# aalto-speech/AaltoASR

Hardware: AMD Instinct MI355X
Metric: frames/sec GMM log-lik (39-d, 50k Gauss) + MFCC, 1/2/4/8 MI355X (higher is better)
Workload: dtype f32 (2-term fp16 split on the matrix cores, f32 accumulate); 1 GPU; configs[2]: full MFCC chain (FFT -> mel -> log -> DCT -> delta/delta-delta, CMS, normalisation) + 50000-Gaussian scoring + 2-byte LNA codes on 1 h of synthetic 16 kHz audio as 360 x 10 s utterances (449280 frames), int16 samples resident in HBM; dim=39, gaussians=50000, states=3125, gpus_flag=1

## Files before the change

aaltoasr_amd/capi.py:

```python
from __future__ import annotations

import ctypes as C
import os
import re
from typing import Optional

import numpy as np

HERE = os.path.dirname(os.path.abspath(__file__))
LIB_PATH = os.path.join(os.environ.get("AASR_LIBDIR") or os.path.join(HERE, "lib"), "libaasr.so")
HEADER_PATH = os.path.join(HERE, "..", "include", "aasr.h")

AASR_OK = 0
AASR_ERR_INVALID = -1
AASR_ERR_UNSUPPORTED = -2
AASR_ERR_NO_DEVICE = -3
AASR_ERR_IO = -4
AASR_ERR_SHORT_AUDIO = -5


class AasrError(RuntimeError):
    def __init__(self, code: int, msg: str):
        super().__init__("aasr status %d: %s" % (code, msg))
        self.code = code
# ... 368 lines not shown
    L.aasr_gmm_score_f64.argtypes = [vp, vp, i64, vp]
    L.aasr_gmm_get_precision.argtypes = [vp]
    L.aasr_gmm_effective_precision.argtypes = [vp]
    L.aasr_gmm_precision_states.argtypes = [vp, C.POINTER(i64), C.POINTER(i64)]
    L.aasr_free.argtypes = [vp]
    L.aasr_free.restype = None
    L.aasr_feat_get_parameters.argtypes = [vp, cp, C.POINTER(C.c_void_p), C.POINTER(i64)]
    L.aasr_feat_num_modules.argtypes = [vp]
    L.aasr_feat_module_name.argtypes = [vp, C.c_int]
    L.aasr_feat_module_name.restype = cp
    L.aasr_feat_module_type.argtypes = [vp, C.c_int]
    L.aasr_feat_module_type.restype = cp
    L.aasr_gmm_score_pitch_ok.argtypes = [vp]
    L.aasr_gmm_score_dev_pitched.argtypes = [vp, vp, i64, vp, i64, vp]
    L.aasr_lna_encode_dev_pitched.argtypes = [vp, i64, i64, i32, C.c_int, C.c_int, vp, vp, vp]
    L.aasr_feat_write_config.argtypes = [vp, C.POINTER(C.c_void_p), C.POINTER(i64)]
    L.aasr_recipe_read.argtypes = [cp, i32, i32, C.POINTER(C.c_void_p), C.POINTER(i64)]
    L.aasr_recipe_read_all.argtypes = [cp, i32, i32, i32, C.POINTER(C.c_void_p), C.POINTER(i64)]
    L.aasr_audio_read.argtypes = [vp, cp, C.POINTER(C.POINTER(C.c_int16)), C.POINTER(i64),
                                  C.POINTER(i32)]


def check(status: int) -> None:
    if status != AASR_OK:
        raise AasrError(status, lib().aasr_last_error().decode("utf-8", "replace"))


def _ptr(a) -> int:
    if a is None:
        return None
# ... 245 lines not shown
                                       _stream_handle(stream)))

    def score_scratch_floats(self, F: int) -> int:
        return lib().aasr_gmm_score_scratch_floats(self._h, F)

    def score_lna_dev(self, d_frames, d_scratch, d_bytes, normalize: bool = True, lnabytes: int = 2, stream=None) -> None:
        check(lib().aasr_gmm_score_lna_dev(self._h, d_frames.data_ptr(), d_frames.shape[0], int(normalize), lnabytes,
                                           d_scratch.data_ptr(), d_bytes.data_ptr(), _stream_handle(stream)))

    def score_pitch_ok(self) -> bool:
        return bool(lib().aasr_gmm_score_pitch_ok(self._h))

    def score_dev_pitched(self, d_frames, d_out, pitch: int, stream=None) -> None:
        check(lib().aasr_gmm_score_dev_pitched(self._h, _ptr(d_frames), d_frames.shape[0], _ptr(d_out),
                                               pitch, _stream_handle(stream)))

    def gauss_loglik(self, frames: np.ndarray) -> np.ndarray:
        frames = np.ascontiguousarray(frames, np.float32)
        self._check_frames(frames)
        out = np.empty((frames.shape[0], self.num_gaussians), np.float32)
        check(lib().aasr_gmm_gauss_loglik(self._h, _ptr(frames), frames.shape[0], _ptr(out)))
        return out


def lna_encode(state_loglik: np.ndarray, normalize: bool = True, lnabytes: int = 2):
    x = np.ascontiguousarray(state_loglik, np.float32)
    F, S = x.shape
    lp = np.empty((F, S), np.float32)
    by = np.empty((F, S * lnabytes), np.uint8)
    check(lib().aasr_lna_encode(_ptr(x), F, S, int(normalize), lnabytes, _ptr(lp), _ptr(by)))
# ... 1707 lines not shown
```

aaltoasr_amd/csrc/capi.cc:

```cpp
#include <cstdarg>
#include <cstdlib>
#include <cstring>
#include <vector>

#include "common.h"
#include "feat.h"
#include "gmm.h"
#include "pipeline.h"

namespace aasr {

std::string &last_error() {
  static thread_local std::string msg;
  return msg;
}

aasr_status fail(aasr_status code, const char *fmt, ...) {
  char buf[1024];
  va_list ap;
  va_start(ap, fmt);
  vsnprintf(buf, sizeof buf, fmt, ap);
  va_end(ap);
  last_error() = buf;
  return code;
// ... 440 lines not shown
  });
}

int aasr_gmm_score_pitch_ok(const aasr_gmm *h) { return h && gmm_score_pitch_ok(h) ? 1 : 0; }

aasr_status aasr_gmm_score_dev_pitched(aasr_gmm *h, const float *d_frames, int64_t F,
                                       float *d_state_loglik, int64_t pitch, void *stream) {
  return guarded([&] {
    if (!h || (F > 0 && (!d_frames || !d_state_loglik)))
      raise(AASR_ERR_INVALID, "aasr_gmm_score_dev_pitched: null argument");
    if (pitch < h->S) raise(AASR_ERR_INVALID, "aasr_gmm_score_dev_pitched: pitch %ld < %ld states", (long)pitch, (long)h->S);
    gmm_score_launch_pitched(h, d_frames, F, d_state_loglik, pitch, (hipStream_t)stream);
  });
}

aasr_status aasr_lna_encode(const float *state_loglik, int64_t F, int32_t S, int normalize,
                            int lnabytes, float *lp_out, uint8_t *bytes_out) {
  return guarded([&] {
    if (lnabytes != 2 && lnabytes != 4)
      raise(AASR_ERR_INVALID, "lnabytes must be 2 or 4, got %d", lnabytes);
    if (S <= 0) raise(AASR_ERR_INVALID, "aasr_lna_encode: S must be positive");
    if (F <= 0) return;
    if (!state_loglik) raise(AASR_ERR_INVALID, "aasr_lna_encode: null input");
    require_device();
    size_t n = (size_t)F * S;
    DevBuf<float> d_in, d_lp;
    DevBuf<uint8_t> d_by;
    d_in.upload(state_loglik, n);
    if (lp_out) d_lp.alloc(n);
    if (bytes_out) d_by.alloc(n * lnabytes);
// ... 68 lines not shown
```

aaltoasr_amd/csrc/gmm.h:

```cpp
#pragma once
#include <cmath>
#include <cstdint>
#include <string>
#include <functional>
#include <memory>
#include <vector>

#include "common.h"

namespace aasr {

struct HostModel {
  int dim = 0;
  int64_t G = 0;
  std::vector<double> mean, var;
  std::vector<double> cov;
  std::vector<uint8_t> is_full;
  bool any_full() const { return !is_full.empty(); }
  std::vector<double> gauss_bias;
  int n_transforms = 0;
  std::vector<int32_t> g2t;
  std::vector<double> xform;
  double logw_bias = 0;
  double logw(size_t k) const {
// ... 264 lines not shown
  aasr::DevBuf<float> dim_part_x, dim_part_ll;
  aasr::DevBuf<int32_t> dim_mix_off, dim_mix_idx;
  aasr::DevBuf<float> dim_mix_logw;
  std::unique_ptr<aasr_gmm> pool_view;
  std::vector<std::unique_ptr<aasr_gmm>> class_models;
  std::vector<aasr::DevBuf<double>> class_a, class_b;
  std::vector<double> class_logdet;
  aasr::DevBuf<float> class_scratch, class_xframes;
  std::shared_ptr<void> utt_scratch;
  std::shared_ptr<void> recipe_scratch;
  aasr::DevBuf<double> xf_a, xf_b;
  aasr::DevBuf<float> d_xframes;
  aasr::ClusterState cl;
  aasr::DevBuf<float> d_frames, d_out;
  mutable aasr::DevBuf<uint32_t> fop_scratch;
};

namespace aasr {
void gmm_build(aasr_gmm *g, const HostModel &m);
void gmm_set_transforms(aasr_gmm *g, int32_t n_transforms, const int32_t *gauss_to_transform, const double *W);
void gmm_build_pool(aasr_gmm *g);
void gmm_dim_split_score(aasr_gmm *g, const float *d_frames, int64_t F, float *d_out, bool per_gaussian, hipStream_t stream,
                         const unsigned long long *maskw = nullptr, int c1 = 0, const int32_t *gclus = nullptr,
                         bool frames_adapted = false);
void gmm_build_pool_centred(aasr_gmm *g);
void gmm_build_f64(aasr_gmm *g, bool any_dim = false);
void gmm_cluster_score_f64_launch(aasr_gmm *g, const double *d_frames, const double *d_members, int64_t F,
                                  double *d_out, int linear, double det, hipStream_t stream);
void gmm_f64_masked_launch(aasr_gmm *g, const double *d_members, int64_t F, double *d_out, int linear, double det,
                           const int32_t *crow, const unsigned long long *maskw, int c1, const double *ll64,
// ... 6 lines not shown
void gmm_build_tracks(aasr_gmm *g, bool grouped);
void gmm_probe_f16x2(aasr_gmm *g);
void gmm_plan_engine_parts(aasr_gmm *g);
bool gmm_engine_parts_active(const aasr_gmm *g);
bool gmm_engine_parts_clustered(const aasr_gmm *g);
void gmm_scatter_columns(const float *dense, int64_t F, int64_t n, float *out, int64_t pitch, hipStream_t stream);
void gmm_add_bias_nofloor(float *d_out, int64_t n, float bias, hipStream_t stream);
void gmm_gather_engine_columns(const aasr_gmm *g, const float *rows, int64_t F, int64_t in_pitch, float *out, int64_t out_pitch,
                               hipStream_t stream);
int64_t gmm_engine_pitch(const aasr_gmm *g);
int64_t gmm_engine_pitch_max(const aasr_gmm *g);
const int32_t *gmm_engine_colmap(const aasr_gmm *g);
void gmm_score_launch_engine(aasr_gmm *g, const float *d_frames, int64_t F, float *d_out, int64_t pitch, hipStream_t stream);
void lna_encode_launch(const float *d_loglik, int64_t F, int S, int normalize, int lnabytes, float *d_lp,
                       uint8_t *d_bytes, hipStream_t stream, int64_t in_pitch, const int32_t *d_colmap = nullptr);
void gmm_build_centred(aasr_gmm *g);
void gmm_build_fullcov(aasr_gmm *g);
void gmm_full_launch(aasr_gmm *g, const float *d_frames, int64_t F, float *d_out,
                     hipStream_t stream);
bool gmm_score_pitch_ok(const aasr_gmm *g);
void gmm_score_launch_pitched(aasr_gmm *g, const float *d_frames, int64_t F, float *d_out, int64_t pitch,
                              hipStream_t stream);
void gmm_score_launch(aasr_gmm *g, const float *d_frames, int64_t F,
                      float *d_out, hipStream_t stream);
void gmm_gauss_launch(aasr_gmm *g, const float *d_frames, int64_t F,
                      float *d_out, hipStream_t stream);
void gmm_set_clustering(aasr_gmm *g, int32_t n_clusters, int64_t n_pairs,
                        const int32_t *gauss_index, const int32_t *cluster_index);
void gmm_read_clustering(aasr_gmm *g, const char *path);
void gmm_set_clustering_min_evals(aasr_gmm *g, double min_clusters, double min_gaussians);
// ... 18 lines not shown
```

aaltoasr_amd/csrc/gmm_score.hip:

```cpp
#include <hip/hip_runtime.h>
#include <mutex>
#include <unordered_map>

#include <cmath>
#include <cstdlib>

#include "gmm_score_common.h"

namespace aasr {

static bool launch_bf16(const aasr_gmm *g, const TrackLayout &L, const float *d_frames, int64_t F,
                        float *d_out, hipStream_t stream, const ClusterArgs *cl = nullptr, int64_t pitch = 0) {
  if (g->precision == AASR_PREC_F16X2 && L.a16h.p && launch_split<2>(g, L, d_frames, F, d_out, stream, cl, pitch))
    return true;
  return launch_split<3>(g, L, d_frames, F, d_out, stream, cl, pitch);
}

namespace {
struct ProbeCache {
  std::mutex mu;
  std::unordered_map<uint64_t, std::vector<int32_t>> verdicts;
  int64_t runs = 0, hits = 0;
};
ProbeCache &probe_cache() {
// ... 431 lines not shown

static bool engine_parts_public(const aasr_gmm *g);
bool gmm_score_pitch_ok(const aasr_gmm *g) {
  if (!g->dim_parts.empty()) return false;
  if (engine_parts_public(g)) return true;
  if (g->cl.enabled && gmm_engine_parts_clustered(g)) return true;
  if (g->host.factor_path() || g->class_routing || g->precision == AASR_PREC_F64) return false;
  if (g->hyb_enabled && g->cl.enabled) return false;
  if (g->ill_conditioned) return g->centred_ok && !g->cl.enabled && (g->layout_mask & 4);
  if (g->cl.enabled && !gmm_cluster_pitch_ok(g)) return false;
  if ((g->layout_mask & 3) != 3) return false;
  const TrackLayout &L = g->paired.ok ? g->paired : g->tracks;
  return (g->precision == AASR_PREC_F32 || g->precision == AASR_PREC_BF16X3 || g->precision == AASR_PREC_F16X2) && L.ok;
}

bool gmm_engine_parts_active(const aasr_gmm *g) {
  return !g->engine_parts.empty() && g->precision == AASR_PREC_F16X2 && g->use_bf16x3 && !g->cl.enabled &&
         !g->class_routing && g->dim_parts.empty() && (g->layout_mask & 3) == 3;
}

bool gmm_engine_parts_clustered(const aasr_gmm *g) {
  return !g->engine_parts.empty() && g->cl.enabled && g->precision == AASR_PREC_F16X2 && g->use_bf16x3 && !g->class_routing &&
         g->dim_parts.empty() && (g->layout_mask & 3) == 3;
}

static bool engine_parts_public(const aasr_gmm *g) {
  if (!gmm_engine_parts_active(g)) return false;
  static const int force_sc = AASR_EXPERIMENT_ENV("AASR_EXP_FORCE_SC") ? atoi(AASR_EXPERIMENT_ENV("AASR_EXP_FORCE_SC")) : 0;
  if (force_sc) return true;
  const TrackLayout &L = g->paired.ok ? g->paired : g->tracks;
// ... 389 lines not shown
```

aaltoasr_amd/csrc/gmm_score_bf16x3.hip:

```cpp
#include "gmm_score_pl.h"

namespace aasr {

template <int NK16, bool GROUPED, bool CL, bool WIDE, int NS>
__global__ __launch_bounds__(WIDE ? 512 : 256, WIDE ? 1 : 2) void k_gmm_diag_score_bf16x3(
    const float *__restrict__ frames, int64_t F, int dim, const float *__restrict__ pivot,
    const uint16_t *__restrict__ apack, const int32_t *__restrict__ split_row,
    const uint16_t *__restrict__ close_mask, const int32_t *__restrict__ sid, int sid_stride,
    float *__restrict__ out, int64_t S, int64_t pitch, float ref_ln, int dbg, ClusterArgs cl) {
  static_assert(NS == 3, "k_gmm_diag_score_bf16x3 is instantiated for the three-term form only");
  extern __shared__ __attribute__((aligned(16))) char smem_raw[];
  constexpr int OG = Bf16Smem<NK16, GROUPED, WIDE, NS>::OG;
  constexpr int kTileBytes = Bf16Smem<NK16, GROUPED, WIDE, NS>::kTileBytes;
  constexpr int kTileFloats = kTileBytes / 4;
  constexpr int kOS = Bf16Smem<NK16, GROUPED, WIDE, NS>::kOutStride;
  constexpr int NW = WIDE ? 8 : 4;
  constexpr int NBUF = WIDE ? 3 : 2;
  constexpr int JMID = NS == 2 ? 1 : (NK16 + 1) / 2;
  constexpr int NAB = NS == 2 ? 2 : 1;
  float *abuf0 = (float *)smem_raw;
  const int tid = threadIdx.x;
  const int wave = tid >> 6;
  const int lane = tid & 63;
  const int group = WIDE ? __builtin_amdgcn_readfirstlane(wave >> 2) : 0;
// ... 287 lines not shown
  if (!attr_set[g->device & 63]) {
    AASR_HIP(hipFuncSetAttribute((const void *)kern, hipFuncAttributeMaxDynamicSharedMemorySize, smem));
    attr_set[g->device & 63] = true;
  }
  const int R = pick_row_cuts(blocks, (WIDE ? 1.0 : 2.0) * (g->num_cus > 0 ? g->num_cus : 256),
                              L.rows_padded / TILE_ROWS, L.max_splits, 6.0);
  const int32_t *split_row = L.splits.p + (size_t)(R - 1) * (L.split_cap + 1) * 4;
  hipLaunchKernelGGL(kern, dim3((unsigned)blocks, (unsigned)R), dim3(NW * 64), smem, stream, d_frames, F,
                     g->dim, g->d_pivot.p, NS == 3 ? L.a16.p : L.a16h.p, split_row, L.close.p, L.sid.p, L.sid_stride,
                     d_out, g->S, pitch, L.ref_ln - (float)g->out_bias_ln, dbg, cl);
  AASR_HIP(hipGetLastError());
}

template bool launch_split<3>(const aasr_gmm *, const TrackLayout &, const float *, int64_t, float *, hipStream_t,
                              const ClusterArgs *, int64_t);

}
```

aaltoasr_amd/csrc/gmm_score_common.h:

```cpp
#pragma once
#include <hip/hip_runtime.h>

#include <cmath>
#include <cstdlib>

#include "gmm.h"

namespace aasr {

typedef float f32x16 __attribute__((ext_vector_type(16)));
typedef float f32x4 __attribute__((ext_vector_type(4)));
typedef float f32x2 __attribute__((ext_vector_type(2)));

#define LN2_F 0.69314718055994530942f
#define LOG2E_F 1.4426950408889634074f
#define LOG_TINY_F (-115.12925464970228f)
#define NEG_BIG_F (-3.0e38f)
#ifndef AASR_ABLATION
#define AASR_ABLATION 0
#endif
#if AASR_ABLATION
#define AASR_DBG(bits) (dbg & (bits))
#else
#define AASR_DBG(bits) false
// ... 116 lines not shown
  int c1 = 0;
  int64_t n_words = 1;
  float floor_val = LOG_TINY_F;
  int64_t n_recs = 0;
};

template <int MODE>
void launch_diag(const aasr_gmm *g, const PackedRows &pr, const float *d_frames,
                 int64_t F, float *d_out, int64_t out_cols, hipStream_t stream);
bool launch_tracks(const aasr_gmm *g, const TrackLayout &L, const float *d_frames, int64_t F,
                   float *d_out, hipStream_t stream, const ClusterArgs *cl = nullptr,
                   int64_t pitch = 0);
template <int NS>
bool launch_split(const aasr_gmm *g, const TrackLayout &L, const float *d_frames, int64_t F,
                  float *d_out, hipStream_t stream, const ClusterArgs *cl = nullptr, int64_t pitch = 0);
extern double g_score_pass_bytes;
bool launch_centred_ops(const aasr_gmm *g, const CentredOps &ops, int dimp, const float *d_frames,
                        int64_t F, float *d_out, hipStream_t stream);
bool launch_centred(const aasr_gmm *g, const float *d_frames, int64_t F, float *d_out,
                    hipStream_t stream, int64_t pitch = 0);
void score_outliers(aasr_gmm *g, const float *d_frames, int64_t F, float *d_out, hipStream_t stream,
                    const int32_t *crow = nullptr, const unsigned long long *maskw = nullptr, int c1 = 0,
                    int64_t n_words = 1, int64_t pitch = 0);
bool hyb_fuse_begin(aasr_gmm *g, const TrackLayout &L, const float *d_frames, int64_t F, hipStream_t stream);
void score_f64_for_f32_callers(aasr_gmm *g, const float *d_frames, int64_t F, float *d_out, hipStream_t stream);

}
```

aaltoasr_amd/csrc/gmm_score_f16x2.hip:

```cpp
#include "gmm_score_common.h"

#ifdef AASR_PL_TRACE
#define AASR_PL_TRACE_UNIT 1
namespace aasr {
__device__ unsigned long long g_pl_trace[8][12];
}
#endif

#include "gmm_score_pl.h"

namespace aasr {

template bool launch_split<2>(const aasr_gmm *, const TrackLayout &, const float *, int64_t, float *, hipStream_t,
                              const ClusterArgs *, int64_t);

extern "C" double aasr_debug_frame_operand_ms(aasr_gmm *g, const float *d_frames, int64_t F, int reps, void *stream_v) {
  if (!g || F <= 0 || reps <= 0) return -1.0;
  hipStream_t stream = (hipStream_t)stream_v;
  const TrackLayout &L = g->paired.ok ? g->paired : g->tracks;
  if (!L.ok || !g->use_bf16x3 || g->precision != AASR_PREC_F16X2 || !L.a16h.p || g->cl.enabled) return -1.0;
  const int NW = F >= 8192 ? 8 : 4;
  const int64_t blocks64 = (F + NW * FRAMES_PER_WAVE - 1) / (NW * FRAMES_PER_WAVE) * NW;
  hipEvent_t e0, e1;
  if (hipEventCreate(&e0) != hipSuccess || hipEventCreate(&e1) != hipSuccess) return -1.0;
  int64_t stride = 0;
  frame_operand<2>(g, L, d_frames, F, blocks64, stream, &stride);
  (void)hipEventRecord(e0, stream);
  for (int i = 0; i < reps; i++) frame_operand<2>(g, L, d_frames, F, blocks64, stream, &stride);
  (void)hipEventRecord(e1, stream);
  (void)hipEventSynchronize(e1);
  float ms = 0;
  (void)hipEventElapsedTime(&ms, e0, e1);
  (void)hipEventDestroy(e0);
  (void)hipEventDestroy(e1);
  return (double)ms / reps;
}
}

#ifdef AASR_PL_TRACE
extern "C" int aasr_debug_pl_trace(unsigned long long *out) {
  if (hipDeviceSynchronize() != hipSuccess) return -1;
  return hipMemcpyFromSymbol(out, HIP_SYMBOL(aasr::g_pl_trace), sizeof(unsigned long long) * 96) == hipSuccess ? 0 : -1;
}
#endif
```

aaltoasr_amd/csrc/gmm_score_pl.h:

```cpp
#pragma once
#include "gmm_score_common.h"

namespace aasr {

struct CutPlan {
  int n_main = 0;
  int blocks_main = 1;
  int blocks_rem = 1;
  int r_main = 1, r_rem = 0;
  const int32_t *split_rem = nullptr;
};

struct PivotGroups {
  const int32_t *colend = nullptr;
  int64_t fop_stride = 0;
  const float *pivots = nullptr;
  const float *tabs = nullptr;
  int sc = 0;
  const uint32_t *hyb_tab = nullptr;
  const float *hyb_part = nullptr;
  int64_t hyb_pitch = 0;
  float hyb_bias = 0.0f;
};

// ... 699 lines not shown
  const bool multi = L.n_pg > 1;
  const CutPlan plan = pick_cut_plan(blocks, (WIDE ? 1.0 : 2.0) * (g->num_cus > 0 ? g->num_cus : 256),
                                     L.rows_padded / TILE_ROWS, L.max_splits, 3.0, L.splits.p, multi ? L.n_pg : 1, L.split_cap);
  PivotGroups pg;
  if constexpr (GROUPED && NS == 2) {
    static const int pgf_env = AASR_EXPERIMENT_ENV("AASR_PGF") ? atoi(AASR_EXPERIMENT_ENV("AASR_PGF")) : 1;
    if (multi && pgf_env && L.pg_tab.p) {
      pg.colend = L.pg_colend.p;
      pg.pivots = L.pg_pivot.p;
      pg.tabs = L.pg_tab.p;
      pg.sc = L.sc ? 1 : 0;
      launch_pl_instance<NK16, GROUPED, CL, WIDE, NS, true, false>(g, L, d_frames, F, d_out, stream, cl, pitch, nullptr, plan, pg);
      return;
    }
  }
  const u32x4 *fop = frame_operand<NS>(g, L, d_frames, F, blocks * NW, stream, &pg.fop_stride);
  if (multi) pg.colend = L.pg_colend.p;
  if constexpr (GROUPED && NS == 2 && !CL) {
    if (!multi && g->hyb_fuse.part && g->hyb_tab.p) {
      pg.hyb_tab = g->hyb_tab.p;
      pg.hyb_part = g->hyb_fuse.part;
      pg.hyb_pitch = g->hyb_fuse.pitch;
      pg.hyb_bias = (float)g->out_bias_ln;
      g->hyb_fuse.used = true;
      g->hyb_fused_launches++;
      launch_pl_instance<NK16, GROUPED, CL, WIDE, NS, false, true>(g, L, d_frames, F, d_out, stream, cl, pitch, fop, plan, pg);
      return;
    }
  }
  launch_pl_instance<NK16, GROUPED, CL, WIDE, NS, false, false>(g, L, d_frames, F, d_out, stream, cl, pitch, fop, plan, pg);
}
// ... 24 lines not shown
}

template <int N, int NS>
static void launch_split_n(const aasr_gmm *g, const TrackLayout &L, const float *d_frames, int64_t F, float *d_out,
                           hipStream_t stream, const ClusterArgs *cl, int64_t pitch, bool wide) {
  const ClusterArgs none;
  if (cl && NS == 2 && wide && wide_ok<N, NS>()) {
    if constexpr (NS == 2) launch_split_tracks<N, NS, true, true>(g, L, d_frames, F, d_out, stream, *cl, pitch);
  } else if (cl) {
    launch_split_tracks<N, NS, true, false>(g, L, d_frames, F, d_out, stream, *cl, pitch);
  } else if (wide && wide_ok<N, NS>()) {
    launch_split_tracks<N, NS, false, true>(g, L, d_frames, F, d_out, stream, none, pitch);
  } else {
    launch_split_tracks<N, NS, false, false>(g, L, d_frames, F, d_out, stream, none, pitch);
  }
}

template <int NS>
bool launch_split(const aasr_gmm *g, const TrackLayout &L, const float *d_frames, int64_t F,
                  float *d_out, hipStream_t stream, const ClusterArgs *cl, int64_t pitch) {
  if (pitch <= 0) pitch = g->S;
  if (NS == 3 ? !L.a16.p : !L.a16h.p) return false;
  static const int wide_env = AASR_EXPERIMENT_ENV("AASR_BF16_WIDE") ? atoi(AASR_EXPERIMENT_ENV("AASR_BF16_WIDE")) : -1;
  const bool wide = (wide_env >= 0 ? wide_env : (F >= 8192 ? 1 : 0)) != 0;
  switch (L.nk16) {
    case 1: launch_split_n<1, NS>(g, L, d_frames, F, d_out, stream, cl, pitch, wide); return true;
    case 2: launch_split_n<2, NS>(g, L, d_frames, F, d_out, stream, cl, pitch, wide); return true;
    case 3: launch_split_n<3, NS>(g, L, d_frames, F, d_out, stream, cl, pitch, wide); return true;
    case 4: launch_split_n<4, NS>(g, L, d_frames, F, d_out, stream, cl, pitch, wide); return true;
    case 5: launch_split_n<5, NS>(g, L, d_frames, F, d_out, stream, cl, pitch, wide); return true;
// ... 8 lines not shown
```

aaltoasr_amd/csrc/lna_encode.hip:

```cpp
#include <hip/hip_runtime.h>

#include <algorithm>
#include <cmath>
#include <cstdlib>

#include "common.h"
#include "lna_device.h"

namespace aasr {

__global__ __launch_bounds__(256) void k_state_norm_lna(
    const float *__restrict__ loglik, int64_t F, int S, int64_t in_pitch, int normalize,
    int lnabytes, float *__restrict__ lp_out, uint8_t *__restrict__ bytes_out) {
  __shared__ double red[8];
  const int tid = threadIdx.x, wave = tid >> 6, lane = tid & 63;
  for (int64_t f = blockIdx.x; f < F; f += gridDim.x) {
    const float *row = loglik + f * in_pitch;
    double logz = 0.0;
    if (normalize) {
      double m = -INFINITY;
      for (int i = tid; i < S; i += 256) {
        double v = float_cast_loglik(row[i]);
        m = v > m ? v : m;
      }
// ... 31 lines not shown
          if ((double)lp < -36.008) {
            code = 0xffff;
          } else {
            int temp = (int)(-1820.0 * (double)lp + .5);
            unsigned b0 = (temp >> 8) & 255, b1 = temp & 255;
            code = (unsigned short)(b0 | (b1 << 8));
          }
          ((unsigned short *)bytes_out)[o] = code;
        }
      }
    }
  }
}


template <int VPT>
__global__ __launch_bounds__(256) void k_state_norm_lna_reg(
    const float *__restrict__ loglik, int64_t F, int S, int64_t in_pitch, int normalize, int lnabytes,
    float *__restrict__ lp_out, uint8_t *__restrict__ bytes_out, const int32_t *__restrict__ colmap) {
  __shared__ double red[8];
  const int tid = threadIdx.x, wave = tid >> 6, lane = tid & 63;
  constexpr int JSAFE = VPT == 4 ? 0 : VPT == 8 ? 4 : VPT == 10 ? 8 : VPT == 13 ? 10 : VPT == 16 ? 13 : 0;
  int col[VPT];
#pragma unroll
  for (int j = 0; j < VPT; j++) {
    const int i = tid + 256 * j;
    col[j] = (colmap && (j < JSAFE || i < S)) ? colmap[i] : i;
  }
  float vn[VPT];
  {
    const float *row = loglik + (int64_t)blockIdx.x * in_pitch;
#pragma unroll
    for (int j = 0; j < VPT; j++) {
      const int i = tid + 256 * j;
      vn[j] = ((j < JSAFE || i < S) && (int64_t)blockIdx.x < F) ? row[col[j]] : -INFINITY;
    }
  }
  for (int64_t f = blockIdx.x; f < F; f += gridDim.x) {
    float v[VPT];
#pragma unroll
    for (int j = 0; j < VPT; j++) v[j] = vn[j];
    if (f + gridDim.x < F) {
      const float *row = loglik + (f + gridDim.x) * in_pitch;
#pragma unroll
      for (int j = 0; j < VPT; j++) {
        const int i = tid + 256 * j;
        vn[j] = (j < JSAFE || i < S) ? row[col[j]] : -INFINITY;
      }
    }
    lna_row_from_registers<VPT, JSAFE>(v, S, tid, wave, lane, red, normalize, lnabytes, f, true, lp_out, bytes_out);
  }
}

__global__ __launch_bounds__(256) void k_state_norm_lna_f64(const double *__restrict__ lik, int64_t F, int S,
                                                            int normalize, int lnabytes, float *__restrict__ lp_out,
                                                            uint8_t *__restrict__ bytes_out) {
  __shared__ double red[4];
  const int tid = threadIdx.x, wave = tid >> 6, lane = tid & 63;
  for (int64_t f = blockIdx.x; f < F; f += gridDim.x) {
    const double *row = lik + f * (int64_t)S;
    double z = 1.0;
    if (normalize) {
// ... 12 lines not shown
      const float lp = (float)(q < 1e-50 ? LOG_TINY_D : log(q));
      lna_store(lp, lnabytes, f * (int64_t)S + i, lp_out, bytes_out);
    }
  }
}

void lna_encode_f64_launch(const double *d_lik, int64_t F, int S, int normalize, int lnabytes, float *d_lp,
                           uint8_t *d_bytes, hipStream_t stream) {
  if (F <= 0 || S <= 0) return;
  const int64_t blocks = std::min<int64_t>(F, 8192);
  hipLaunchKernelGGL(k_state_norm_lna_f64, dim3((unsigned)blocks), dim3(256), 0, stream, d_lik, F, S, normalize, lnabytes,
                     d_lp, d_bytes);
  AASR_HIP(hipGetLastError());
}

void lna_encode_launch(const float *d_loglik, int64_t F, int S, int normalize,
                       int lnabytes, float *d_lp, uint8_t *d_bytes, hipStream_t stream, int64_t in_pitch,
                       const int32_t *d_colmap) {
  if (in_pitch <= 0) in_pitch = S;
  if (F <= 0 || S <= 0) return;
  if (d_colmap && S > 256 * 16) raise(AASR_ERR_UNSUPPORTED, "a column map needs the register-resident LNA kernels (S <= 4096)");
  int64_t blocks = F < (1 << 20) ? F : (1 << 20);
  int dev = 0, cus = 256;
  if (hipGetDevice(&dev) == hipSuccess) (void)hipDeviceGetAttribute(&cus, hipDeviceAttributeMultiprocessorCount, dev);
  if (S <= 256 * 16) blocks = std::min<int64_t>(blocks, (int64_t)cus * 32);
  if (S <= 256 * 4)
    hipLaunchKernelGGL(k_state_norm_lna_reg<4>, dim3((unsigned)blocks), dim3(256), 0, stream,
                       d_loglik, F, S, in_pitch, normalize, lnabytes, d_lp, d_bytes, d_colmap);
  else if (S <= 256 * 8)
    hipLaunchKernelGGL(k_state_norm_lna_reg<8>, dim3((unsigned)blocks), dim3(256), 0, stream,
                       d_loglik, F, S, in_pitch, normalize, lnabytes, d_lp, d_bytes, d_colmap);
  else if (S <= 256 * 10)
    hipLaunchKernelGGL(k_state_norm_lna_reg<10>, dim3((unsigned)blocks), dim3(256), 0, stream,
                       d_loglik, F, S, in_pitch, normalize, lnabytes, d_lp, d_bytes, d_colmap);
  else if (S <= 256 * 13)
    hipLaunchKernelGGL(k_state_norm_lna_reg<13>, dim3((unsigned)blocks), dim3(256), 0, stream,
                       d_loglik, F, S, in_pitch, normalize, lnabytes, d_lp, d_bytes, d_colmap);
  else if (S <= 256 * 16)
    hipLaunchKernelGGL(k_state_norm_lna_reg<16>, dim3((unsigned)blocks), dim3(256), 0, stream,
                       d_loglik, F, S, in_pitch, normalize, lnabytes, d_lp, d_bytes, d_colmap);
  else
    hipLaunchKernelGGL(k_state_norm_lna, dim3((unsigned)blocks), dim3(256), 0, stream, d_loglik,
                       F, S, in_pitch, normalize, lnabytes, d_lp, d_bytes);
  AASR_HIP(hipGetLastError());
}

}
```

aaltoasr_amd/pipeline.py:

```python
from __future__ import annotations

import os

import numpy as np

from . import capi, synth

class FullChainBench:
    def __init__(self, gmm: capi.Gmm, n_utts: int, seconds: float, rank: int, device,
                 cfg_text: str = None, lnabytes: int = 2, utts=None):
        import torch
        self.torch = torch
        self.gmm = gmm
        self.cfg_text = cfg_text if cfg_text is not None else synth.make_feature_config()
        self.feat = capi.Feat(self.cfg_text)
        self.lnabytes = lnabytes
        sr = self.feat.sample_rate
        n = int(round(seconds * sr))
        if utts is None:
            base = [synth.make_audio(n, seed=synth.SEED + 1000 * rank + i, sample_rate=sr) for i in range(8)]
            utts = [base[i % len(base)] for i in range(n_utts)]
        self.utts = utts
        frames = [self.feat.eof_frame(len(u)) for u in utts]
        self.pcm_off = np.concatenate([[0], np.cumsum([len(u) for u in utts])]).astype(np.int64)
        self.frame_off = np.concatenate([[0], np.cumsum(frames)]).astype(np.int64)
        self.total_frames = int(self.frame_off[-1])
        self.d_pcm = torch.from_numpy(np.concatenate(utts)).to(device)
        S = gmm.num_states
        self.d_fea = torch.empty((self.total_frames, self.feat.dim), dtype=torch.float32, device=device)
        self.S = S
        self.pitch = (S + 31) // 32 * 32 if gmm.score_pitch_ok() else S
        self.d_ll = torch.empty((self.total_frames, self.pitch), dtype=torch.float32, device=device)
        self.d_bytes = torch.empty((self.total_frames, S * lnabytes), dtype=torch.uint8, device=device)
        self.stream = torch.cuda.current_stream()

    def step(self) -> None:
        self.feat.run_batch_dev(self.d_pcm, self.pcm_off, self.frame_off, self.d_fea, self.stream)
        self.gmm.score_dev_pitched(self.d_fea, self.d_ll, self.pitch, self.stream)
        capi.lna_encode_dev(self.d_ll, True, self.lnabytes, None, self.d_bytes, self.stream, num_states=self.S)

    def score_only(self) -> None:
        self.gmm.score_dev_pitched(self.d_fea, self.d_ll, self.pitch, self.stream)

    def features_only(self) -> None:
        self.feat.run_batch_dev(self.d_pcm, self.pcm_off, self.frame_off, self.d_fea, self.stream)

    def lna_only(self) -> None:
        capi.lna_encode_dev(self.d_ll, True, self.lnabytes, None, self.d_bytes, self.stream, num_states=self.S)

    def stage_split(self, reps: int = 3) -> dict:
        torch = self.torch
        out = {}
        for name, fn in (("features", self.features_only), ("scoring", self.score_only), ("lna", self.lna_only)):
            e0, e1 = torch.cuda.Event(enable_timing=True), torch.cuda.Event(enable_timing=True)
# ... 17 lines not shown
```

include/aasr.h:

```cpp
#ifndef AASR_H
#define AASR_H

#include <stddef.h>
#include <stdint.h>

#ifdef __cplusplus
extern "C" {
#endif

typedef int aasr_status;
enum {
  AASR_OK = 0,
  AASR_ERR_INVALID = -1,
  AASR_ERR_UNSUPPORTED = -2,
  AASR_ERR_NO_DEVICE = -3,
  AASR_ERR_IO = -4,
  AASR_ERR_SHORT_AUDIO = -5
};

typedef struct aasr_feat aasr_feat;
typedef struct aasr_gmm aasr_gmm;

const char *aasr_last_error(void);
const char *aasr_version(void);
// ... 113 lines not shown
aasr_status aasr_gmm_gauss_loglik_dev(aasr_gmm *h, const float *d_frames,
                                      int64_t F, float *d_gauss_loglik,
                                      void *stream);


aasr_status aasr_lna_encode(const float *state_loglik, int64_t F, int32_t S,
                            int normalize, int lnabytes, float *lp_out,
                            uint8_t *bytes_out);
aasr_status aasr_lna_encode_dev_pitched(const float *d_state_loglik, int64_t in_pitch, int64_t F,
                                        int32_t S, int normalize, int lnabytes, float *d_lp_out,
                                        uint8_t *d_bytes_out, void *stream);
aasr_status aasr_lna_encode_dev(const float *d_state_loglik, int64_t F,
                                int32_t S, int normalize, int lnabytes,
                                float *d_lp_out, uint8_t *d_bytes_out,
                                void *stream);
int64_t aasr_gmm_score_scratch_floats(const aasr_gmm *h, int64_t F);
aasr_status aasr_gmm_score_lna_dev(aasr_gmm *h, const float *d_frames, int64_t F, int normalize, int lnabytes,
                                   float *d_scratch, uint8_t *d_bytes_out, void *stream);

void aasr_lna_header(int32_t num_states, int lnabytes, uint8_t out[5]);

aasr_status aasr_lna_read_file(const char *path, int32_t *num_states, int32_t *lnabytes, int64_t *frames,
                               float **log_probs);


aasr_status aasr_recipe_batch_range(int32_t num_lines_total, int32_t num_batches,
                                    int32_t batch_index, int32_t *first_line,
                                    int32_t *num_lines);

aasr_status aasr_recipe_read(const char *recipe_text, int32_t num_batches, int32_t batch_index,
// ... 602 lines not shown
```

Baseline: 42.51 million frames/s.

## Overlap chunked GMM scoring with LNA encoding on a side stream

Splits scoring into frame chunks sized to one round of CUs and launches the LNA encode for each chunk on a separate non-blocking stream, synchronised by events, so quantisation overlaps with the next chunk's matrix-core scoring. The fp16-split frame operand is now formed once for all frames up front and reused by each chunk launch instead of being rebuilt per call. The LNA kernel also gets a compile-time variant that skips column-map loads when no map is given. The extra launches, event syncs and concurrent kernels competing for CUs may cancel out the overlap.

```diff
diff --git a/aaltoasr_amd/capi.py b/aaltoasr_amd/capi.py
--- a/aaltoasr_amd/capi.py
+++ b/aaltoasr_amd/capi.py
@@ -406,6 +406,9 @@
     L.aasr_gmm_score_pitch_ok.argtypes = [vp]
     L.aasr_gmm_score_dev_pitched.argtypes = [vp, vp, i64, vp, i64, vp]
     L.aasr_lna_encode_dev_pitched.argtypes = [vp, i64, i64, i32, C.c_int, C.c_int, vp, vp, vp]
+    L.aasr_gmm_score_lna_pitched_dev.argtypes = [vp, vp, i64, vp, i64, C.c_int, C.c_int, vp, i64, vp]
+    L.aasr_gmm_score_lna_overlap_active.argtypes = [vp, i64, i64, i64]
+    L.aasr_gmm_score_lna_overlap_active.restype = C.c_int
     L.aasr_feat_write_config.argtypes = [vp, C.POINTER(C.c_void_p), C.POINTER(i64)]
     L.aasr_recipe_read.argtypes = [cp, i32, i32, C.POINTER(C.c_void_p), C.POINTER(i64)]
     L.aasr_recipe_read_all.argtypes = [cp, i32, i32, i32, C.POINTER(C.c_void_p), C.POINTER(i64)]
@@ -681,6 +684,15 @@
     def score_dev_pitched(self, d_frames, d_out, pitch: int, stream=None) -> None:
         check(lib().aasr_gmm_score_dev_pitched(self._h, _ptr(d_frames), d_frames.shape[0], _ptr(d_out),
                                                pitch, _stream_handle(stream)))
+
+    def score_lna_dev_pitched(self, d_frames, d_scores, pitch: int, d_bytes, normalize: bool = True, lnabytes: int = 2,
+                              chunk_frames: int = 0, stream=None) -> None:
+        check(lib().aasr_gmm_score_lna_pitched_dev(self._h, _ptr(d_frames), d_frames.shape[0], _ptr(d_scores), pitch,
+                                                   int(normalize), lnabytes, _ptr(d_bytes), chunk_frames,
+                                                   _stream_handle(stream)))
+
+    def score_lna_overlap_active(self, n_frames: int, pitch: int, chunk_frames: int = 0) -> bool:
+        return bool(lib().aasr_gmm_score_lna_overlap_active(self._h, n_frames, pitch, chunk_frames))
 
     def gauss_loglik(self, frames: np.ndarray) -> np.ndarray:
         frames = np.ascontiguousarray(frames, np.float32)
diff --git a/aaltoasr_amd/csrc/capi.cc b/aaltoasr_amd/csrc/capi.cc
--- a/aaltoasr_amd/csrc/capi.cc
+++ b/aaltoasr_amd/csrc/capi.cc
@@ -478,6 +478,24 @@
   });
 }
 
+aasr_status aasr_gmm_score_lna_pitched_dev(aasr_gmm *h, const float *d_frames, int64_t F, float *d_scores, int64_t pitch,
+                                           int normalize, int lnabytes, uint8_t *d_bytes, int64_t chunk_frames,
+                                           void *stream) {
+  return guarded([&] {
+    if (!h || (F > 0 && (!d_frames || !d_scores || !d_bytes)))
+      raise(AASR_ERR_INVALID, "aasr_gmm_score_lna_pitched_dev: null argument");
+    if (lnabytes != 2 && lnabytes != 4) raise(AASR_ERR_INVALID, "lnabytes must be 2 or 4, got %d", lnabytes);
+    if (pitch < h->S) raise(AASR_ERR_INVALID, "aasr_gmm_score_lna_pitched_dev: pitch %ld < %ld states", (long)pitch, (long)h->S);
+    gmm_score_lna_chunked(h, d_frames, F, d_scores, pitch, normalize, lnabytes, d_bytes, chunk_frames, (hipStream_t)stream);
+  });
+}
+
+int aasr_gmm_score_lna_overlap_active(const aasr_gmm *h, int64_t F, int64_t pitch, int64_t chunk_frames) {
+  int active = 0;
+  if (h && F > 0 && pitch >= h->S) (void)guarded([&] { active = gmm_score_lna_chunk(h, F, pitch, chunk_frames) > 0 ? 1 : 0; });
+  return active;
+}
+
 aasr_status aasr_lna_encode(const float *state_loglik, int64_t F, int32_t S, int normalize,
                             int lnabytes, float *lp_out, uint8_t *bytes_out) {
   return guarded([&] {
diff --git a/aaltoasr_amd/csrc/gmm.h b/aaltoasr_amd/csrc/gmm.h
--- a/aaltoasr_amd/csrc/gmm.h
+++ b/aaltoasr_amd/csrc/gmm.h
@@ -302,6 +302,13 @@
   aasr::ClusterState cl;
   aasr::DevBuf<float> d_frames, d_out;
   mutable aasr::DevBuf<uint32_t> fop_scratch;
+  std::shared_ptr<void> score_lna_side;
+  struct FopAhead {
+    const float *frames = nullptr;
+    int64_t F = 0, stride = 0;
+    int ns = 0;
+  };
+  mutable FopAhead fop_ahead;
 };
 
 namespace aasr {
@@ -338,6 +345,13 @@
 void gmm_score_launch_engine(aasr_gmm *g, const float *d_frames, int64_t F, float *d_out, int64_t pitch, hipStream_t stream);
 void lna_encode_launch(const float *d_loglik, int64_t F, int S, int normalize, int lnabytes, float *d_lp,
                        uint8_t *d_bytes, hipStream_t stream, int64_t in_pitch, const int32_t *d_colmap = nullptr);
+bool gmm_score_single_track_launch(const aasr_gmm *g, int64_t pitch);
+int gmm_score_frame_operand_terms(const aasr_gmm *g);
+void gmm_form_frame_operand(aasr_gmm *g, const float *d_frames, int64_t F, hipStream_t stream);
+void gmm_drop_frame_operand(const aasr_gmm *g);
+int64_t gmm_score_lna_chunk(const aasr_gmm *g, int64_t F, int64_t pitch, int64_t chunk_frames);
+void gmm_score_lna_chunked(aasr_gmm *g, const float *d_frames, int64_t F, float *d_scores, int64_t pitch, int normalize,
+                           int lnabytes, uint8_t *d_bytes, int64_t chunk_frames, hipStream_t stream);
 void gmm_build_centred(aasr_gmm *g);
 void gmm_build_fullcov(aasr_gmm *g);
 void gmm_full_launch(aasr_gmm *g, const float *d_frames, int64_t F, float *d_out,
diff --git a/aaltoasr_amd/csrc/gmm_score.hip b/aaltoasr_amd/csrc/gmm_score.hip
--- a/aaltoasr_amd/csrc/gmm_score.hip
+++ b/aaltoasr_amd/csrc/gmm_score.hip
@@ -469,6 +469,35 @@
   return (g->precision == AASR_PREC_F32 || g->precision == AASR_PREC_BF16X3 || g->precision == AASR_PREC_F16X2) && L.ok;
 }
 
+bool gmm_score_single_track_launch(const aasr_gmm *g, int64_t pitch) {
+  if (pitch < g->S || !g->dim_parts.empty() || g->cl.enabled || g->class_routing || g->host.factor_path()) return false;
+  if (g->precision != AASR_PREC_F32 && g->precision != AASR_PREC_BF16X3 && g->precision != AASR_PREC_F16X2) return false;
+  if (gmm_engine_parts_active(g) || g->ill_conditioned || g->hyb_enabled || g->xf_a.p) return false;
+  if ((g->layout_mask & 3) != 3) return false;
+  const TrackLayout &L = g->paired.ok ? g->paired : g->tracks;
+  if (!L.ok || L.n_pg > 1) return false;
+  return pitch == g->S || gmm_score_pitch_ok(g);
+}
+
+int gmm_score_frame_operand_terms(const aasr_gmm *g) {
+  if (!g->use_bf16x3) return 0;
+  const TrackLayout &L = g->paired.ok ? g->paired : g->tracks;
+  if (!L.ok || L.n_pg > 1) return 0;
+  if (L.nk16 < 1 || L.nk16 == 7 || L.nk16 > 8) return 0;
+  if (g->precision == AASR_PREC_F16X2 && L.a16h.p) return 2;
+  return L.a16.p && L.nk16 <= 5 ? 3 : 0;
+}
+
+void gmm_form_frame_operand(aasr_gmm *g, const float *d_frames, int64_t F, hipStream_t stream) {
+  const TrackLayout &L = g->paired.ok ? g->paired : g->tracks;
+  const int ns = gmm_score_frame_operand_terms(g);
+  if (ns == 2) form_frame_operand<2>(g, L, d_frames, F, stream);
+  else if (ns == 3) form_frame_operand<3>(g, L, d_frames, F, stream);
+  else g->fop_ahead = aasr_gmm::FopAhead();
+}
+
+void gmm_drop_frame_operand(const aasr_gmm *g) { g->fop_ahead = aasr_gmm::FopAhead(); }
+
 bool gmm_engine_parts_active(const aasr_gmm *g) {
   return !g->engine_parts.empty() && g->precision == AASR_PREC_F16X2 && g->use_bf16x3 && !g->cl.enabled &&
          !g->class_routing && g->dim_parts.empty() && (g->layout_mask & 3) == 3;
diff --git a/aaltoasr_amd/csrc/gmm_score_bf16x3.hip b/aaltoasr_amd/csrc/gmm_score_bf16x3.hip
--- a/aaltoasr_amd/csrc/gmm_score_bf16x3.hip
+++ b/aaltoasr_amd/csrc/gmm_score_bf16x3.hip
@@ -325,5 +325,6 @@
 
 template bool launch_split<3>(const aasr_gmm *, const TrackLayout &, const float *, int64_t, float *, hipStream_t,
                               const ClusterArgs *, int64_t);
+template void form_frame_operand<3>(const aasr_gmm *, const TrackLayout &, const float *, int64_t, hipStream_t);
 
 }
diff --git a/aaltoasr_amd/csrc/gmm_score_common.h b/aaltoasr_amd/csrc/gmm_score_common.h
--- a/aaltoasr_amd/csrc/gmm_score_common.h
+++ b/aaltoasr_amd/csrc/gmm_score_common.h
@@ -154,6 +154,8 @@
 template <int NS>
 bool launch_split(const aasr_gmm *g, const TrackLayout &L, const float *d_frames, int64_t F,
                   float *d_out, hipStream_t stream, const ClusterArgs *cl = nullptr, int64_t pitch = 0);
+template <int NS>
+void form_frame_operand(const aasr_gmm *g, const TrackLayout &L, const float *d_frames, int64_t F, hipStream_t stream);
 extern double g_score_pass_bytes;
 bool launch_centred_ops(const aasr_gmm *g, const CentredOps &ops, int dimp, const float *d_frames,
                         int64_t F, float *d_out, hipStream_t stream);
diff --git a/aaltoasr_amd/csrc/gmm_score_f16x2.hip b/aaltoasr_amd/csrc/gmm_score_f16x2.hip
--- a/aaltoasr_amd/csrc/gmm_score_f16x2.hip
+++ b/aaltoasr_amd/csrc/gmm_score_f16x2.hip
@@ -13,6 +13,7 @@
 
 template bool launch_split<2>(const aasr_gmm *, const TrackLayout &, const float *, int64_t, float *, hipStream_t,
                               const ClusterArgs *, int64_t);
+template void form_frame_operand<2>(const aasr_gmm *, const TrackLayout &, const float *, int64_t, hipStream_t);
 
 extern "C" double aasr_debug_frame_operand_ms(aasr_gmm *g, const float *d_frames, int64_t F, int reps, void *stream_v) {
   if (!g || F <= 0 || reps <= 0) return -1.0;
@@ -35,6 +36,10 @@
   (void)hipEventDestroy(e1);
   return (double)ms / reps;
 }
+
+extern "C" int aasr_debug_pl_bench_smem_bytes(int wide) {
+  return wide ? PlSmem<5, true, true, 2>::kBytes : PlSmem<5, true, false, 2>::kBytes;
+}
 }
 
 #ifdef AASR_PL_TRACE
diff --git a/aaltoasr_amd/csrc/gmm_score_lna.cc b/aaltoasr_amd/csrc/gmm_score_lna.cc
--- /dev/null
+++ b/aaltoasr_amd/csrc/gmm_score_lna.cc
@@ -0,0 +1,82 @@
+#include <algorithm>
+#include <memory>
+
+#include "gmm.h"
+
+namespace aasr {
+
+namespace {
+
+constexpr int kEvents = 8;
+
+struct SideStream {
+  hipStream_t side = nullptr;
+  hipEvent_t scored[kEvents] = {};
+  hipEvent_t lna_done = nullptr;
+  ~SideStream() {
+    if (side) (void)hipStreamSynchronize(side);
+    for (hipEvent_t e : scored)
+      if (e) (void)hipEventDestroy(e);
+    if (lna_done) (void)hipEventDestroy(lna_done);
+    if (side) (void)hipStreamDestroy(side);
+  }
+};
+
+SideStream *side_of(aasr_gmm *g) {
+  if (!g->score_lna_side) {
+    auto s = std::make_shared<SideStream>();
+    AASR_HIP(hipStreamCreateWithFlags(&s->side, hipStreamNonBlocking));
+    for (hipEvent_t &e : s->scored) AASR_HIP(hipEventCreateWithFlags(&e, hipEventDisableTiming));
+    AASR_HIP(hipEventCreateWithFlags(&s->lna_done, hipEventDisableTiming));
+    g->score_lna_side = s;
+  }
+  return static_cast<SideStream *>(g->score_lna_side.get());
+}
+
+struct Join {
+  const aasr_gmm *g;
+  SideStream *ss;
+  hipStream_t stream;
+  ~Join() {
+    gmm_drop_frame_operand(g);
+    if (hipEventRecord(ss->lna_done, ss->side) == hipSuccess) (void)hipStreamWaitEvent(stream, ss->lna_done, 0);
+  }
+};
+
+}
+
+int64_t gmm_score_lna_chunk(const aasr_gmm *g, int64_t F, int64_t pitch, int64_t chunk_frames) {
+  if (chunk_frames < 0 || chunk_frames % 512 != 0)
+    raise(AASR_ERR_INVALID, "chunk_frames must be 0 or a positive multiple of 512, got %ld", (long)chunk_frames);
+  if (!gmm_score_single_track_launch(g, pitch)) return 0;
+  if (chunk_frames > 0) return F > chunk_frames ? chunk_frames : 0;
+  const int64_t round = (int64_t)(g->num_cus > 0 ? g->num_cus : 256) * 512;
+  return F >= 2 * round ? round : 0;
+}
+
+void gmm_score_lna_chunked(aasr_gmm *g, const float *d_frames, int64_t F, float *d_scores, int64_t pitch, int normalize,
+                           int lnabytes, uint8_t *d_bytes, int64_t chunk_frames, hipStream_t stream) {
+  const int64_t chunk = gmm_score_lna_chunk(g, F, pitch, chunk_frames);
+  if (F <= 0) return;
+  const int S = (int)g->S;
+  if (chunk == 0) {
+    gmm_score_launch_pitched(g, d_frames, F, d_scores, pitch, stream);
+    lna_encode_launch(d_scores, F, S, normalize, lnabytes, nullptr, d_bytes, stream, pitch);
+    return;
+  }
+  SideStream *ss = side_of(g);
+  Join join{g, ss, stream};
+  gmm_form_frame_operand(g, d_frames, F, stream);
+  int c = 0;
+  for (int64_t f0 = 0; f0 < F; f0 += chunk, c++) {
+    const int64_t n = std::min(chunk, F - f0);
+    gmm_score_launch_pitched(g, d_frames + f0 * g->dim, n, d_scores + f0 * pitch, pitch, stream);
+    hipEvent_t e = ss->scored[c % kEvents];
+    AASR_HIP(hipEventRecord(e, stream));
+    AASR_HIP(hipStreamWaitEvent(ss->side, e, 0));
+    lna_encode_launch(d_scores + f0 * pitch, n, S, normalize, lnabytes, nullptr, d_bytes + (size_t)f0 * S * lnabytes,
+                      ss->side, pitch);
+  }
+}
+
+}
diff --git a/aaltoasr_amd/csrc/gmm_score_pl.h b/aaltoasr_amd/csrc/gmm_score_pl.h
--- a/aaltoasr_amd/csrc/gmm_score_pl.h
+++ b/aaltoasr_amd/csrc/gmm_score_pl.h
@@ -737,7 +737,19 @@
       return;
     }
   }
-  const u32x4 *fop = frame_operand<NS>(g, L, d_frames, F, blocks * NW, stream, &pg.fop_stride);
+  const u32x4 *fop = nullptr;
+  const aasr_gmm::FopAhead &ah = g->fop_ahead;
+  if (!multi && ah.frames && ah.ns == NS && d_frames >= ah.frames) {
+    const int64_t off = d_frames - ah.frames, unit = (int64_t)512 * g->dim;
+    if (off % unit == 0 && off / g->dim + F <= ah.F) {
+      fop = (const u32x4 *)g->fop_scratch.p + (size_t)(off / g->dim / 64) * ((size_t)L.nk16 * NS * 2 * 64);
+      pg.fop_stride = ah.stride;
+    }
+  }
+  if (!fop) {
+    g->fop_ahead = aasr_gmm::FopAhead();
+    fop = frame_operand<NS>(g, L, d_frames, F, blocks * NW, stream, &pg.fop_stride);
+  }
   if (multi) pg.colend = L.pg_colend.p;
   if constexpr (GROUPED && NS == 2 && !CL) {
     if (!multi && g->hyb_fuse.part && g->hyb_tab.p) {
@@ -792,6 +804,18 @@
   } else {
     launch_split_tracks<N, NS, false, false>(g, L, d_frames, F, d_out, stream, none, pitch);
   }
+}
+
+template <int NS>
+void form_frame_operand(const aasr_gmm *g, const TrackLayout &L, const float *d_frames, int64_t F, hipStream_t stream) {
+  g->fop_ahead = aasr_gmm::FopAhead();
+  if (F <= 0 || L.n_pg > 1) return;
+  int64_t stride = 0;
+  frame_operand<NS>(g, L, d_frames, F, (F + 511) / 512 * 8, stream, &stride);
+  g->fop_ahead.frames = d_frames;
+  g->fop_ahead.F = F;
+  g->fop_ahead.stride = stride;
+  g->fop_ahead.ns = NS;
 }
 
 template <int NS>
diff --git a/aaltoasr_amd/csrc/lna_encode.hip b/aaltoasr_amd/csrc/lna_encode.hip
--- a/aaltoasr_amd/csrc/lna_encode.hip
+++ b/aaltoasr_amd/csrc/lna_encode.hip
@@ -69,18 +69,20 @@
 }
 
 
-template <int VPT>
+template <int VPT, bool MAPPED>
 __global__ __launch_bounds__(256) void k_state_norm_lna_reg(
     const float *__restrict__ loglik, int64_t F, int S, int64_t in_pitch, int normalize, int lnabytes,
     float *__restrict__ lp_out, uint8_t *__restrict__ bytes_out, const int32_t *__restrict__ colmap) {
   __shared__ double red[8];
   const int tid = threadIdx.x, wave = tid >> 6, lane = tid & 63;
   constexpr int JSAFE = VPT == 4 ? 0 : VPT == 8 ? 4 : VPT == 10 ? 8 : VPT == 13 ? 10 : VPT == 16 ? 13 : 0;
-  int col[VPT];
+  int col[MAPPED ? VPT : 1];
+  if constexpr (MAPPED) {
 #pragma unroll
-  for (int j = 0; j < VPT; j++) {
-    const int i = tid + 256 * j;
-    col[j] = (colmap && (j < JSAFE || i < S)) ? colmap[i] : i;
+    for (int j = 0; j < VPT; j++) {
+      const int i = tid + 256 * j;
+      col[j] = (colmap && (j < JSAFE || i < S)) ? colmap[i] : i;
+    }
   }
   float vn[VPT];
   {
@@ -88,7 +90,7 @@
 #pragma unroll
     for (int j = 0; j < VPT; j++) {
       const int i = tid + 256 * j;
-      vn[j] = ((j < JSAFE || i < S) && (int64_t)blockIdx.x < F) ? row[col[j]] : -INFINITY;
+      vn[j] = ((j < JSAFE || i < S) && (int64_t)blockIdx.x < F) ? row[MAPPED ? col[j] : i] : -INFINITY;
     }
   }
   for (int64_t f = blockIdx.x; f < F; f += gridDim.x) {
@@ -100,7 +102,7 @@
 #pragma unroll
       for (int j = 0; j < VPT; j++) {
         const int i = tid + 256 * j;
-        vn[j] = (j < JSAFE || i < S) ? row[col[j]] : -INFINITY;
+        vn[j] = (j < JSAFE || i < S) ? row[MAPPED ? col[j] : i] : -INFINITY;
       }
     }
     lna_row_from_registers<VPT, JSAFE>(v, S, tid, wave, lane, red, normalize, lnabytes, f, true, lp_out, bytes_out);
@@ -143,6 +145,17 @@
   AASR_HIP(hipGetLastError());
 }
 
+template <int VPT>
+static void launch_lna_reg(unsigned blocks, hipStream_t stream, const float *d_loglik, int64_t F, int S, int64_t in_pitch,
+                           int normalize, int lnabytes, float *d_lp, uint8_t *d_bytes, const int32_t *d_colmap) {
+  if (d_colmap)
+    hipLaunchKernelGGL((k_state_norm_lna_reg<VPT, true>), dim3(blocks), dim3(256), 0, stream, d_loglik, F, S, in_pitch,
+                       normalize, lnabytes, d_lp, d_bytes, d_colmap);
+  else
+    hipLaunchKernelGGL((k_state_norm_lna_reg<VPT, false>), dim3(blocks), dim3(256), 0, stream, d_loglik, F, S, in_pitch,
+                       normalize, lnabytes, d_lp, d_bytes, d_colmap);
+}
+
 void lna_encode_launch(const float *d_loglik, int64_t F, int S, int normalize,
                        int lnabytes, float *d_lp, uint8_t *d_bytes, hipStream_t stream, int64_t in_pitch,
                        const int32_t *d_colmap) {
@@ -153,23 +166,19 @@
   int dev = 0, cus = 256;
   if (hipGetDevice(&dev) == hipSuccess) (void)hipDeviceGetAttribute(&cus, hipDeviceAttributeMultiprocessorCount, dev);
   if (S <= 256 * 16) blocks = std::min<int64_t>(blocks, (int64_t)cus * 32);
+  const unsigned nb = (unsigned)blocks;
   if (S <= 256 * 4)
-    hipLaunchKernelGGL(k_state_norm_lna_reg<4>, dim3((unsigned)blocks), dim3(256), 0, stream,
-                       d_loglik, F, S, in_pitch, normalize, lnabytes, d_lp, d_bytes, d_colmap);
+    launch_lna_reg<4>(nb, stream, d_loglik, F, S, in_pitch, normalize, lnabytes, d_lp, d_bytes, d_colmap);
   else if (S <= 256 * 8)
-    hipLaunchKernelGGL(k_state_norm_lna_reg<8>, dim3((unsigned)blocks), dim3(256), 0, stream,
-                       d_loglik, F, S, in_pitch, normalize, lnabytes, d_lp, d_bytes, d_colmap);
+    launch_lna_reg<8>(nb, stream, d_loglik, F, S, in_pitch, normalize, lnabytes, d_lp, d_bytes, d_colmap);
   else if (S <= 256 * 10)
-    hipLaunchKernelGGL(k_state_norm_lna_reg<10>, dim3((unsigned)blocks), dim3(256), 0, stream,
-                       d_loglik, F, S, in_pitch, normalize, lnabytes, d_lp, d_bytes, d_colmap);
+    launch_lna_reg<10>(nb, stream, d_loglik, F, S, in_pitch, normalize, lnabytes, d_lp, d_bytes, d_colmap);
   else if (S <= 256 * 13)
-    hipLaunchKernelGGL(k_state_norm_lna_reg<13>, dim3((unsigned)blocks), dim3(256), 0, stream,
-                       d_loglik, F, S, in_pitch, normalize, lnabytes, d_lp, d_bytes, d_colmap);
+    launch_lna_reg<13>(nb, stream, d_loglik, F, S, in_pitch, normalize, lnabytes, d_lp, d_bytes, d_colmap);
   else if (S <= 256 * 16)
-    hipLaunchKernelGGL(k_state_norm_lna_reg<16>, dim3((unsigned)blocks), dim3(256), 0, stream,
-                       d_loglik, F, S, in_pitch, normalize, lnabytes, d_lp, d_bytes, d_colmap);
+    launch_lna_reg<16>(nb, stream, d_loglik, F, S, in_pitch, normalize, lnabytes, d_lp, d_bytes, d_colmap);
   else
-    hipLaunchKernelGGL(k_state_norm_lna, dim3((unsigned)blocks), dim3(256), 0, stream, d_loglik,
+    hipLaunchKernelGGL(k_state_norm_lna, dim3(nb), dim3(256), 0, stream, d_loglik,
                        F, S, in_pitch, normalize, lnabytes, d_lp, d_bytes);
   AASR_HIP(hipGetLastError());
 }
diff --git a/aaltoasr_amd/pipeline.py b/aaltoasr_amd/pipeline.py
--- a/aaltoasr_amd/pipeline.py
+++ b/aaltoasr_amd/pipeline.py
@@ -36,8 +36,7 @@
 
     def step(self) -> None:
         self.feat.run_batch_dev(self.d_pcm, self.pcm_off, self.frame_off, self.d_fea, self.stream)
-        self.gmm.score_dev_pitched(self.d_fea, self.d_ll, self.pitch, self.stream)
-        capi.lna_encode_dev(self.d_ll, True, self.lnabytes, None, self.d_bytes, self.stream, num_states=self.S)
+        self.gmm.score_lna_dev_pitched(self.d_fea, self.d_ll, self.pitch, self.d_bytes, True, self.lnabytes, 0, self.stream)
 
     def score_only(self) -> None:
         self.gmm.score_dev_pitched(self.d_fea, self.d_ll, self.pitch, self.stream)
diff --git a/include/aasr.h b/include/aasr.h
--- a/include/aasr.h
+++ b/include/aasr.h
@@ -151,6 +151,10 @@
                                 int32_t S, int normalize, int lnabytes,
                                 float *d_lp_out, uint8_t *d_bytes_out,
                                 void *stream);
+aasr_status aasr_gmm_score_lna_pitched_dev(aasr_gmm *h, const float *d_frames, int64_t F, float *d_scores, int64_t pitch,
+                                           int normalize, int lnabytes, uint8_t *d_bytes, int64_t chunk_frames,
+                                           void *stream);
+int aasr_gmm_score_lna_overlap_active(const aasr_gmm *h, int64_t F, int64_t pitch, int64_t chunk_frames);
 int64_t aasr_gmm_score_scratch_floats(const aasr_gmm *h, int64_t F);
 aasr_status aasr_gmm_score_lna_dev(aasr_gmm *h, const float *d_frames, int64_t F, int normalize, int lnabytes,
                                    float *d_scratch, uint8_t *d_bytes_out, void *stream);
```

Measured after the change: 43.73 million frames/s, median of 6. 2.9% higher.
